# Maxwell-Zhao/RoboSimGS

Measured on AMD Instinct MI355X. Metric: frames/sec + ms/frame (fwd, fwd+bwd) at 1M Gaussians 1920x1080, higher is better.
Workload: dtype f32

## Files before the change

robosimgs_amd/csrc/binning.hip:

```cpp
#include "mgs_common.h"
#include "tile_rect.h"
#include "tile_order.h"

namespace mgs {
namespace {

constexpr int kBlock = 128;

__device__ __forceinline__ uint32_t wave_sum(uint32_t v) {
#pragma unroll
  for (int d = 32; d >= 1; d >>= 1) v += __shfl_xor(v, d);
  return v;
}

constexpr int kSum = 64;
__global__ __launch_bounds__(kBlock) void tile_count_kernel(
    int n, const float* __restrict__ means2d, const int32_t* __restrict__ radii,
    const int32_t* __restrict__ radii_y, const float* __restrict__ conics, const float* __restrict__ opacities,
    float tile_size, int tile_w, int tile_h, uint2* __restrict__ ginfo, uint32_t* __restrict__ sums) {
  int g = blockIdx.x * kBlock + threadIdx.x;
  int radius = g < n ? radii[g] : 0;
  uint2 info = make_uint2(kEmptyTileRect, 0u);
  if (radius > 0) {
    float2 m = reinterpret_cast<const float2*>(means2d)[g];
// ... 319 lines not shown
  uint32_t kept[kColKeep];
  uint32_t sum = 0;
  if (kCanKeep && keep) {
#pragma unroll
    for (int j = 0; j < kColKeep; ++j) {
      if (j >= rpg) { kept[j] = 0u; continue; }
      kept[j] = (ok && r0 + j < r1) ? table[(size_t)(r0 + j) * n_tiles + t] : 0u;
    }
#pragma unroll
    for (int j = 0; j < kColKeep; ++j) sum += kept[j];
  } else {
    for (int r = r0; r < r1; r += 16) {
      uint32_t v[16];
#pragma unroll
      for (int j = 0; j < 16; ++j) v[j] = (ok && r + j < r1) ? table[(size_t)(r + j) * n_tiles + t] : 0u;
#pragma unroll
      for (int j = 0; j < 16; ++j) sum += v[j];
    }
  }
  part[rg][bl] = sum;
  __syncthreads();
  uint32_t off = 0, tot = 0;
#pragma unroll 16
  for (int g = 0; g < kColGroups; ++g) {
    const uint32_t s = part[g][bl];
    if (g < rg) off += s;
    tot += s;
  }
  if (kCanKeep && keep) {
#pragma unroll
    for (int j = 0; j < kColKeep; ++j) {
      if (j >= rpg) continue;
      if (ok && r0 + j < r1) {
        table[(size_t)(r0 + j) * n_tiles + t] = off;
        off += kept[j];
      }
    }
  } else {
    for (int r = r0; r < r1; r += 16) {
      uint32_t v[16];
#pragma unroll
      for (int j = 0; j < 16; ++j) v[j] = (ok && r + j < r1) ? table[(size_t)(r + j) * n_tiles + t] : 0u;
#pragma unroll
      for (int j = 0; j < 16; ++j)
        if (ok && r + j < r1) {
          table[(size_t)(r + j) * n_tiles + t] = off;
          off += v[j];
        }
    }
  }
  if (rg == 0 && ok) tile_count[t] = tot;
}

template <bool PAIRS>
__global__ __launch_bounds__(kDirectThreads) void direct_scatter_kernel(
    int n, int chunk, const uint2* __restrict__ ginfo, int tile_w, int n_tiles, int shift,
    const uint32_t* __restrict__ table, const uint32_t* __restrict__ tile_count, uint32_t capacity,
    uint32_t* __restrict__ flatten_ids, int32_t* __restrict__ tile_offsets,
    uint32_t* __restrict__ n_isect, uint32_t* __restrict__ status, int32_t* __restrict__ group_order,
    const uint32_t* __restrict__ scanned_sums, int4* __restrict__ pair_info, uint32_t* __restrict__ zero_word,
    float* __restrict__ splat_slots, int deal_nb) {
  extern __shared__ uint32_t cursor[];
  n_tiles = (n_tiles + (1 << shift) - 1) >> shift;
  if (group_order && blockIdx.x == gridDim.x - 1) {
    order_groups_by_total<kDirectThreads>(n_tiles, [&](int g) { return tile_count[g]; }, group_order);
    return;
  }
  const uint32_t local_mask = (1u << shift) - 1u;
  __shared__ unsigned long long wsum[kDirectThreads / 64];
  const unsigned lane = threadIdx.x & 63, wave = threadIdx.x >> 6;
  const int per = (n_tiles + kDirectThreads - 1) / kDirectThreads;
  const int t0 = (int)threadIdx.x * per;
  unsigned long long sum = 0;
  for (int k = 0; k < per; ++k)
    if (t0 + k < n_tiles) sum += tile_count[t0 + k];
  unsigned long long incl = sum;
#pragma unroll
  for (int d = 1; d < 64; d <<= 1) {
    const uint32_t lo = __shfl_up((uint32_t)incl, d), hi = __shfl_up((uint32_t)(incl >> 32), d);
    if (lane >= (unsigned)d) incl += ((unsigned long long)hi << 32) | lo;
  }
  if (lane == 63) wsum[wave] = incl;
  __syncthreads();
  unsigned long long off = 0, total = 0;
#pragma unroll
  for (int w = 0; w < kDirectThreads / 64; ++w) {
    if ((unsigned)w < wave) off += wsum[w];
    total += wsum[w];
  }
  unsigned long long ex = off + incl - sum;
  const uint32_t* row = table + (size_t)blockIdx.x * n_tiles;
  for (int k = 0; k < per; ++k) {
    const int t = t0 + k;
    if (t < n_tiles) {
      const uint32_t at = ex < capacity ? (uint32_t)ex : capacity;
      cursor[t] = ex < capacity ? at + row[t] : capacity;
      if (blockIdx.x == 0) tile_offsets[t] = (int32_t)at;
      ex += tile_count[t];
    }
  }
  if (blockIdx.x == 0 && threadIdx.x == 0) {
    tile_offsets[n_tiles] = (int32_t)(total < capacity ? (uint32_t)total : capacity);
    *n_isect = total > 0xffffffffull ? 0xffffffffu : (uint32_t)total;
    *status = total > capacity ? MGS_STATUS_ISECT_OVERFLOW : 0u;
    if (zero_word) reinterpret_cast<uint4*>(zero_word)[0] = reinterpret_cast<uint4*>(zero_word)[1] = make_uint4(0u, 0u, 0u, 0u);
  }
  __syncthreads();
  const int g0 = blockIdx.x * chunk, g1 = min(n, g0 + chunk);
  const DealtIndex gi{g0, g1, n, deal_nb};
  const int g_end = deal_nb > 0 ? g0 + chunk : g1;
  for (int base = g0; base < g_end; base += kDirectThreads * kDirectPerThread) {
    uint2 info[kDirectPerThread];
#pragma unroll
    for (int i = 0; i < kDirectPerThread; ++i) {
      const int g = gi(base, i);
      info[i] = g >= 0 ? ginfo[g] : make_uint2(kEmptyTileRect, 0u);
    }
    if (PAIRS) {
// ... 56 lines not shown
  if (i0 + kOffsetsPerThread <= n) {
    const uint4 a = *reinterpret_cast<const uint4*>(tiles + i0), b = *reinterpret_cast<const uint4*>(tiles + i0 + 4);
    v[0] = a.x; v[1] = a.y; v[2] = a.z; v[3] = a.w; v[4] = b.x; v[5] = b.y; v[6] = b.z; v[7] = b.w;
  } else {
#pragma unroll
    for (int j = 0; j < kOffsetsPerThread; ++j) v[j] = i0 + j < n ? tiles[i0 + j] : 0u;
  }
  int prev = i0 ? (int)tiles[i0 - 1] : -1;
#pragma unroll
  for (int j = 0; j < kOffsetsPerThread; ++j) {
    const uint32_t i = i0 + j;
    if (i < n) {
      const int cur = (int)v[j];
      for (int k = prev + 1; k <= cur; ++k) offsets[k] = (int32_t)i;
      prev = cur;
      if (i == n - 1)
        for (int k = cur + 1; k <= n_tiles; ++k) offsets[k] = (int32_t)n;
    }
  }
}

__global__ __launch_bounds__(kBlock) void isect_ids_kernel(
    const uint32_t* __restrict__ n_ptr, uint32_t capacity, const uint32_t* __restrict__ tiles,
    const int32_t* __restrict__ ids, const float* __restrict__ depths, int64_t cam_shifted,
    int64_t* __restrict__ isect_ids) {
  uint32_t n = min(*n_ptr, capacity);
  uint32_t i = blockIdx.x * kBlock + threadIdx.x;
  if (i >= n) return;
  int64_t hi = cam_shifted | (int64_t)tiles[i];
  isect_ids[i] = (hi << 32) | (int64_t)__float_as_uint(depths[ids[i]]);
}

__global__ __launch_bounds__(kBlock) void offset_encode_kernel(
    uint32_t n, const int64_t* __restrict__ isect_ids, int n_cams, int n_tiles, int tile_bits,
    int32_t* __restrict__ offsets) {
  uint32_t i = blockIdx.x * kBlock + threadIdx.x;
  int total = n_cams * n_tiles;
  if (n == 0) {
    for (uint32_t k = i; k < (uint32_t)total; k += gridDim.x * kBlock) offsets[k] = 0;
    return;
  }
  if (i >= n) return;
  auto flat = [&](int64_t key) {
    int64_t t = key >> 32;
    return (int)((t >> tile_bits) * n_tiles + (t & ((1ll << tile_bits) - 1)));
  };
  int cur = flat(isect_ids[i]);
  int prev = i ? flat(isect_ids[i - 1]) : -1;
  for (int k = prev + 1; k <= cur && k < total; ++k) offsets[k] = (int32_t)i;
  if (i == n - 1)
    for (int k = cur + 1; k < total; ++k) offsets[k] = (int32_t)n;
}

__global__ __launch_bounds__(1024) void tile_group_order_kernel(int n_tiles, const int32_t* __restrict__ tile_offsets,
                                                                int32_t* __restrict__ order) {
  order_groups_by_total<1024>((n_tiles + 3) / 4, [&](int g) {
    return (uint32_t)(tile_offsets[min(4 * g + 4, n_tiles)] - tile_offsets[4 * g]);
  }, order);
}

int bits_for(uint32_t count) {
  int b = 0;
  while (count > 1 && (1ull << b) < count) ++b;
  return b;
}

unsigned direct_chunk(unsigned n) {
  const unsigned per_block = max(div_up(n, kDirectMaxBlocks), (unsigned)(kDirectThreads * kDirectPerThread));
  return div_up(per_block, kDirectThreads) * kDirectThreads;
}
unsigned direct_blocks(unsigned n) { return div_up(n, direct_chunk(n)); }

struct Workspace {
  size_t total;
  size_t ginfo, blocksums, tile_alt, tile_priv, id_alt, radix, tsort, table, tile_count, group_offsets;
  Workspace(int n, uint32_t cap, int n_tiles) {
    Bump b(0);
    size_t nn = (size_t)(n > 0 ? n : 1), cc = cap ? cap : 1;
    ginfo = b.take(nn * 8);
    blocksums = b.take((size_t)div_up((unsigned)nn, kSum) * 4);
    tile_alt = b.take(cc * 4); id_alt = b.take(cc * 4);
    tile_priv = b.take(cc * 4);
    radix = b.take(radix_sort_temp_bytes((uint32_t)cc));
    tsort = b.take(tile_depth_sort_temp_bytes((uint32_t)cc, n_tiles));
    const size_t nt = (size_t)(n_tiles < kDirectMaxTiles ? n_tiles : kDirectMaxTiles);
    table = b.take((size_t)direct_blocks((unsigned)nn) * nt * 4);
    tile_count = b.take(nt * 4);
    group_offsets = b.take((nt + 1) * 4);
    total = b.total;
  }
};

}
}

namespace mgs {
size_t isect_tiles_workspace_bytes(int n, uint32_t capacity, int n_tiles) { return Workspace(n, capacity, n_tiles).total; }

int launch_tile_group_order(int n_tiles, const int32_t* tile_offsets, int32_t* order, hipStream_t stream) {
  hipLaunchKernelGGL(tile_group_order_kernel, dim3(1), dim3(1024), 0, stream, n_tiles, tile_offsets, order);
  return check_launch("tile_group_order");
}
}

using namespace mgs;

extern "C" int mgs_isect_tiles(int n, const float* means2d, const int32_t* radii, const int32_t* radii_y,
                               const float* depths, const float* conics, const float* opacities,
                               int tile_size, int tile_w, int tile_h,
                               int cam_id, int n_cams, uint32_t isect_capacity,
                               int32_t* tiles_per_gauss, uint32_t* n_isect, uint32_t* tile_ids,
                               int32_t* flatten_ids, int64_t* isect_ids, int32_t* tile_offsets,
                               int32_t* pair_info, int32_t* tile_group_order, uint32_t* status,
                               const uint32_t* seed_info,
                               uint32_t* seed_sums, float* splat_slots, void* workspace,
                               size_t* workspace_bytes, mgs_stream_t stream) {
  MGS_REQUIRE(n >= 0 && tile_size > 0 && tile_w > 0 && tile_h > 0, "isect_tiles: bad sizes");
  MGS_REQUIRE(tile_w <= 1023 && tile_h <= 1023, "isect_tiles: tile grid %dx%d exceeds 1023x1023", tile_w, tile_h);
  MGS_REQUIRE(workspace_bytes, "isect_tiles: workspace_bytes is null");
  MGS_REQUIRE(cam_id >= 0 && n_cams > cam_id, "isect_tiles: cam_id %d outside 0..%d", cam_id, n_cams);
  const Workspace ws(n, isect_capacity, tile_w * tile_h);
  if (!workspace) {
    *workspace_bytes = ws.total;
    return MGS_OK;
  }
  if (*workspace_bytes < ws.total)
    return set_error(MGS_ERR_WORKSPACE_TOO_SMALL, "isect_tiles: workspace %zu < %zu bytes",
                     *workspace_bytes, ws.total);
  MGS_REQUIRE(isect_capacity > 0, "isect_tiles: zero capacity");
  MGS_REQUIRE(seed_info || (conics == nullptr) == (opacities == nullptr),
              "isect_tiles: tight tile bounds need both conics and opacities");
  MGS_REQUIRE(n == 0 || (seed_info == nullptr) == (seed_sums == nullptr),
              "isect_tiles: seed_info and seed_sums come together (mgs_project_color_fwd writes both)");
  MGS_REQUIRE((n == 0 || ((seed_info || (means2d && radii)) && depths)) && n_isect && flatten_ids &&
                  tile_offsets && status, "isect_tiles: null pointer");
  MGS_REQUIRE(!seed_info || tile_size == MGS_TILE_SIZE, "isect_tiles: a seed is for tile_size %d, got %d", MGS_TILE_SIZE, tile_size);
  MGS_REQUIRE(!seed_sums || (reinterpret_cast<uintptr_t>(seed_sums) & 15u) == 0, "isect_tiles: seed_sums must be 16-byte aligned");
  MGS_REQUIRE(!splat_slots || pair_info, "isect_tiles: splat_slots are written with pair_info");
  MGS_REQUIRE(!splat_slots || (reinterpret_cast<uintptr_t>(splat_slots) & 15u) == 0, "isect_tiles: splat_slots must be 16-byte aligned");
  hipStream_t s = (hipStream_t)stream;
  char* w = static_cast<char*>(workspace);
  auto u32 = [&](size_t off) { return reinterpret_cast<uint32_t*>(w + off); };
  const bool want_tile_ids = tile_ids != nullptr;
  if (!tile_ids) tile_ids = u32(ws.tile_priv);
  const int n_tiles = tile_w * tile_h;
  const uint32_t cap = isect_capacity;
  const int gshift = (sort_opts() & 8) ? (sort_opts() >> 4) & 7 : kGroupShift;
  const bool direct = ((n_tiles + (1 << gshift) - 1) >> gshift) <= kDirectMaxTiles && !(sort_opts() & 4) &&
                      (gshift == 0 || (unsigned)n <= (1u << (32 - gshift)));
  int rc;
  bool order_done = false;

  if (n == 0) {
    (void)hipMemsetAsync(n_isect, 0, 4, s);
    (void)hipMemsetAsync(status, 0, 4, s);
  } else {
    const unsigned nblk = div_up(n, kBlock), nsum = div_up(n, kSum);
    const uint2* ginfo = reinterpret_cast<const uint2*>(seed_info);
    uint32_t* sums = seed_sums;
    if (!seed_info) {
      uint2* gi = reinterpret_cast<uint2*>(w + ws.ginfo);
      sums = u32(ws.blocksums);
      hipLaunchKernelGGL(tile_count_kernel, dim3(nblk), dim3(kBlock), 0, s, n, means2d, radii, radii_y, conics,
                         opacities, (float)tile_size, tile_w, tile_h, gi, sums);
      ginfo = gi;
    }
    if (direct) {
      const int chunk = (int)direct_chunk((unsigned)n);
      const unsigned nb = direct_blocks((unsigned)n);
      const int bins = (n_tiles + (1 << gshift) - 1) >> gshift;
      const size_t lds = (size_t)bins * sizeof(uint32_t);
      const int deal_nb = (int)nb;
      hipLaunchKernelGGL(direct_hist_kernel, dim3(nb + (pair_info ? 1 : 0)), dim3(kDirectThreads), lds, s, n, chunk, ginfo, tile_w,
                         n_tiles, gshift, u32(ws.table), tiles_per_gauss, pair_info ? sums : nullptr, nsum, deal_nb);
      if (pair_info)
        hipLaunchKernelGGL(direct_colscan_kernel<kColKeepTraining>, dim3(div_up((unsigned)bins, (unsigned)kColBins)), dim3(kColThreads), 0, s,
                           (int)nb, bins, u32(ws.table), u32(ws.tile_count));
      else
        hipLaunchKernelGGL(direct_colscan_kernel<1>, dim3(div_up((unsigned)bins, (unsigned)kColBins)), dim3(kColThreads), 0, s,
                           (int)nb, bins, u32(ws.table), u32(ws.tile_count));
      const bool order_in_scatter = tile_group_order && gshift == 2;
      order_done = order_in_scatter;
      with_bool(pair_info != nullptr, [&](auto training) {
        hipLaunchKernelGGL(direct_scatter_kernel<decltype(training)::value>, dim3(nb + (order_in_scatter ? 1 : 0)),
                           dim3(kDirectThreads), lds, s, n, chunk, ginfo, tile_w, n_tiles, gshift, u32(ws.table),
                           u32(ws.tile_count), cap, gshift ? u32(ws.id_alt) : reinterpret_cast<uint32_t*>(flatten_ids),
                           gshift ? reinterpret_cast<int32_t*>(w + ws.group_offsets) : tile_offsets, n_isect, status,
                           order_in_scatter ? tile_group_order : nullptr, sums, reinterpret_cast<int4*>(pair_info),
                           tile_depth_sort_long_list(w + ws.tsort, cap), pair_info ? splat_slots : nullptr, deal_nb);
      });
    } else {
      hipLaunchKernelGGL(scan_blocksums_kernel, dim3(1), dim3(kScanThreads), 0, s, nsum, sums, cap,
                         n_isect, status);
      const int tile_bits = bits_for((uint32_t)n_tiles);
      const int passes = (tile_bits + 7) / 8;
      uint32_t* user_t = tile_ids;
      uint32_t* user_i = reinterpret_cast<uint32_t*>(flatten_ids);
      uint32_t *a_t = user_t, *a_i = user_i, *b_t = u32(ws.tile_alt), *b_i = u32(ws.id_alt);
      if (passes & 1) { a_t = u32(ws.tile_alt); a_i = u32(ws.id_alt); b_t = user_t; b_i = user_i; }
      hipLaunchKernelGGL(emit_kernel, dim3(nblk), dim3(kBlock), 0, s, n, ginfo, tile_w, sums, cap, a_t,
                         a_i, tiles_per_gauss);
      if (pair_info)
        hipLaunchKernelGGL(pair_info_kernel, dim3(nblk), dim3(kBlock), 0, s, n, ginfo, tile_h, sums,
                           reinterpret_cast<int4*>(pair_info), splat_slots);
      rc = radix_sort_pairs(n_isect, cap, tile_bits, a_t, a_i, b_t, b_i, w + ws.radix, s);
      if (rc) return rc;
    }
  }
  if (!direct || n == 0)
    hipLaunchKernelGGL(tile_offsets_kernel, dim3(div_up(cap, kBlock * kOffsetsPerThread)), dim3(kBlock), 0,
                       s, n_isect, cap, tile_ids, n_tiles, tile_offsets);
  if (n > 0) {
    const bool grouped = direct && gshift > 0;
    rc = tile_depth_sort(n_tiles, tile_offsets, depths, cap, reinterpret_cast<uint32_t*>(flatten_ids),
                         direct && (want_tile_ids || isect_ids) ? tile_ids : nullptr, w + ws.tsort, s,
                          u32(ws.tile_alt), u32(ws.id_alt),
                         grouped ? u32(ws.id_alt) : nullptr,
                         grouped ? reinterpret_cast<const int32_t*>(w + ws.group_offsets) : nullptr, gshift, direct);
    if (rc) return rc;
  }
  if (tile_group_order && !order_done) {
    rc = launch_tile_group_order(n_tiles, tile_offsets, tile_group_order, s);
    if (rc) return rc;
  }
  const unsigned gblk = div_up(cap, kBlock);
  if (isect_ids) {
    const int tile_bits_key = bits_for((uint32_t)n_tiles + 1);
    hipLaunchKernelGGL(isect_ids_kernel, dim3(gblk), dim3(kBlock), 0, s, n_isect, cap, tile_ids,
                       flatten_ids, depths, (int64_t)cam_id << tile_bits_key, isect_ids);
  }
  return check_launch("isect_tiles");
}

extern "C" int mgs_isect_offset_encode(uint32_t n_isect, const int64_t* isect_ids, int n_cams,
                                       int tile_w, int tile_h, int32_t* offsets,
                                       mgs_stream_t stream) {
  MGS_REQUIRE(n_cams > 0 && tile_w > 0 && tile_h > 0, "isect_offset_encode: bad sizes");
  MGS_REQUIRE(offsets && (isect_ids || n_isect == 0), "isect_offset_encode: null pointer");
  const int n_tiles = tile_w * tile_h;
  const int tile_bits = bits_for((uint32_t)n_tiles + 1);
  unsigned gblk = n_isect ? div_up(n_isect, kBlock) : div_up((unsigned)(n_cams * n_tiles), kBlock);
  hipLaunchKernelGGL(offset_encode_kernel, dim3(gblk), dim3(kBlock), 0, (hipStream_t)stream,
                     n_isect, isect_ids, n_cams, n_tiles, tile_bits, offsets);
// ... 3 lines not shown
```

robosimgs_amd/csrc/labels.hip:

```cpp
#include "weight_walk.h"
#include "tile_order.h"
#include "../../include/mgs_labels.h"

namespace mgs {
namespace {

__global__ __launch_bounds__(64) void raster_labels_kernel(
    const float* __restrict__ means2d, const float* __restrict__ conics, const float* __restrict__ opacities,
    const float4* __restrict__ splats, const int32_t* __restrict__ class_ids, int n_classes, int width, int height,
    int tile_w, int n_tiles, const int32_t* __restrict__ tile_offsets, const int32_t* __restrict__ flatten_ids,
    const int32_t* __restrict__ group_order, uint8_t* __restrict__ labels, float* __restrict__ label_weights) {
  __shared__ WeightEntry queue[kQueue + 1];
  extern __shared__ __attribute__((aligned(16))) float class_w[];
  const int tile = tile_of_unit((int)blockIdx.x, n_tiles, group_order);
  if (tile < 0) return;
  const unsigned lane = threadIdx.x & 63u;
  const TileFrame fr = tile_frame(tile, tile_w, lane);
  const int start = tile_offsets[tile], end = tile_offsets[tile + 1];
  const int ix = fr.ix, iy = fr.iy;
  if (start >= end) {
#pragma unroll
    for (int k = 0; k < 4; ++k) {
      const int x = ix + 8 * (k & 1), y = iy + 8 * (k >> 1);
      if (x < width && y < height) {
        const size_t p = (size_t)y * width + x;
        labels[p] = MGS_LABEL_NONE;
        if (label_weights) label_weights[p] = 0.f;
      }
    }
    return;
  }

  for (int i = 0; i < n_classes; ++i)
    reinterpret_cast<float4*>(class_w)[i * 64 + lane] = make_float4(0.f, 0.f, 0.f, 0.f);

  unsigned long long alive[4];
#pragma unroll
  for (int k = 0; k < 4; ++k)
    alive[k] = ballot(ix + 8 * (k & 1) < width && iy + 8 * (k >> 1) < height);
  __builtin_amdgcn_fence(__ATOMIC_RELEASE, "wavefront");
  __builtin_amdgcn_wave_barrier();
  __builtin_amdgcn_fence(__ATOMIC_ACQUIRE, "wavefront");

  weight_walk(queue, fr, lane, start, end, splats, means2d, conics, opacities, flatten_ids, alive,
              [&](int g) { return class_ids[g]; },
              [&](int cls, auto quad) {
                const bool counted = (unsigned)cls < (unsigned)n_classes;
                float* slot = class_w + (counted ? cls : 0) * 256 + lane;
#pragma unroll
                for (int k = 0; k < 4; ++k) {
                  float w;
                  if (quad(k, w) && counted) atomicAdd(slot + 64 * k, w);
                }
              });

  __builtin_amdgcn_fence(__ATOMIC_RELEASE, "wavefront");
  __builtin_amdgcn_wave_barrier();
  __builtin_amdgcn_fence(__ATOMIC_ACQUIRE, "wavefront");
  float best[4] = {0.f, 0.f, 0.f, 0.f};
  int label[4] = {MGS_LABEL_NONE, MGS_LABEL_NONE, MGS_LABEL_NONE, MGS_LABEL_NONE};
  for (int c = 0; c < n_classes; ++c) {
#pragma unroll
    for (int k = 0; k < 4; ++k) {
      const float v = class_w[c * 256 + 64 * k + lane];
      if (v > best[k]) { best[k] = v; label[k] = c; }
    }
  }
#pragma unroll
  for (int k = 0; k < 4; ++k) {
    const int x = ix + 8 * (k & 1), y = iy + 8 * (k >> 1);
    if (x < width && y < height) {
      const size_t p = (size_t)y * width + x;
      labels[p] = (uint8_t)label[k];
      if (label_weights) label_weights[p] = best[k];
    }
  }
}

}

int check_label_args(const char* fn, const int32_t* class_ids, int n_classes, const uint8_t* labels) {
  MGS_REQUIRE(n_classes >= 1 && n_classes <= MGS_LABELS_MAX_CLASSES, "%s: n_classes %d outside 1..%d", fn, n_classes,
              MGS_LABELS_MAX_CLASSES);
  MGS_REQUIRE(class_ids, "%s: class_ids is null", fn);
  MGS_REQUIRE(labels, "%s: labels is null", fn);
  return MGS_OK;
}

}

using namespace mgs;

extern "C" int mgs_raster_labels(int n, const float* means2d, const float* conics, const float* opacities,
                                 const float* splats, const int32_t* class_ids, int n_classes, int width, int height,
                                 int tile_w, int tile_h, const int32_t* tile_offsets, const int32_t* flatten_ids,
                                 const int32_t* tile_group_order, uint8_t* labels, float* label_weights,
                                 mgs_stream_t stream) {
  const int rc = check_label_args("raster_labels", class_ids, n_classes, labels);
  if (rc) return rc;
  MGS_REQUIRE(splats || (means2d && conics && opacities),
              "raster_labels: neither packed records (splats) nor means2d, conics and opacities given");
  MGS_REQUIRE(n >= 0 && width > 0 && height > 0, "raster_labels: bad sizes");
  MGS_REQUIRE(tile_w == (width + 15) / 16 && tile_h == (height + 15) / 16,
              "raster_labels: tile grid %dx%d does not match %dx%d at tile size 16", tile_w, tile_h, width, height);
  MGS_REQUIRE(tile_offsets && flatten_ids, "raster_labels: null tile lists");
  const int n_tiles = tile_w * tile_h, n_units = tile_launch_units(n_tiles, tile_group_order);
  hipLaunchKernelGGL(raster_labels_kernel, dim3(n_units), dim3(64), (size_t)n_classes * 1024, (hipStream_t)stream, means2d,
                     conics, opacities, reinterpret_cast<const float4*>(splats), class_ids, n_classes, width, height, tile_w,
                     n_tiles, tile_offsets, flatten_ids, tile_group_order, labels, label_weights);
  return check_launch("raster_labels");
}
```

robosimgs_amd/csrc/lift.hip:

```cpp
#include "weight_walk.h"
#include "tile_order.h"
#include "../../include/mgs_lift.h"

#include <math.h>

namespace mgs {
namespace {

constexpr float kVoteOne = 4294967296.f;

__global__ __launch_bounds__(64) void raster_votes_kernel(
    const float* __restrict__ means2d, const float* __restrict__ conics, const float* __restrict__ opacities,
    const float4* __restrict__ splats, const uint8_t* __restrict__ mask, int n_classes, int width, int height, int tile_w,
    int n_tiles, const int32_t* __restrict__ tile_offsets, const int32_t* __restrict__ flatten_ids,
    const int32_t* __restrict__ group_order, int row_offset, int n_rows, unsigned long long* __restrict__ votes) {
  __shared__ WeightEntry queue[kQueue + 1];
  const int tile = tile_of_unit((int)blockIdx.x, n_tiles, group_order);
  if (tile < 0) return;
  const unsigned lane = threadIdx.x & 63u;
  const int start = tile_offsets[tile], end = tile_offsets[tile + 1];
  if (start >= end) return;
  const TileFrame fr = tile_frame(tile, tile_w, lane);

  unsigned cls_of[4];
  unsigned have = 0u;
#pragma unroll
  for (int k = 0; k < 4; ++k) {
    const int x = fr.ix + 8 * (k & 1), y = fr.iy + 8 * (k >> 1);
    unsigned m = 255u;
    if (x < width && y < height) m = mask[(size_t)y * width + x];
    if (m >= (unsigned)n_classes) m = 255u;
    else have |= 1u << m;
    cls_of[k] = m;
  }
  const unsigned mask4 = cls_of[0] | cls_of[1] << 8 | cls_of[2] << 16 | cls_of[3] << 24;
  const unsigned present = wave_or(have);
  if (present == 0u) return;

  unsigned long long alive[4];
#pragma unroll
  for (int k = 0; k < 4; ++k) alive[k] = ballot(((mask4 >> (8 * k)) & 255u) != 255u);

  weight_walk(queue, fr, lane, start, end, splats, means2d, conics, opacities, flatten_ids, alive,
              [&](int g) { return g - row_offset; },
              [&](int row, auto quad) {
                float w[4] = {0.f, 0.f, 0.f, 0.f};
#pragma unroll
                for (int k = 0; k < 4; ++k) quad(k, w[k]);
                if ((unsigned)row >= (unsigned)n_rows) return;
                if (ballot((w[0] + w[1]) + (w[2] + w[3]) > 0.f) == 0ull) return;
                unsigned long long* dst = votes + (size_t)row * (size_t)n_classes;
                unsigned todo = present;
                while (todo != 0u) {
                  const unsigned c = (unsigned)__builtin_ctz(todo);
                  todo &= todo - 1u;
                  float s[4];
#pragma unroll
                  for (int k = 0; k < 4; ++k) s[k] = ((mask4 >> (8 * k)) & 255u) == c ? w[k] : 0.f;
                  const float sum = wave_reduce_to_lane63((s[0] + s[1]) + (s[2] + s[3]));
                  if (lane == 63u && sum > 0.f)
                    atomicAdd(dst + c, (unsigned long long)rintf(sum * kVoteOne));
                }
              });
}

__global__ __launch_bounds__(256) void lift_assign_kernel(int n_rows, int n_classes,
                                                          const unsigned long long* __restrict__ votes,
                                                          unsigned long long min_vote, int32_t* __restrict__ class_ids,
                                                          float* __restrict__ confidence) {
  const int g = (int)(blockIdx.x * 256u + threadIdx.x);
  if (g >= n_rows) return;
  const unsigned long long* v = votes + (size_t)g * (size_t)n_classes;
  unsigned long long best = 0ull, total = 0ull;
  int cls = 0;
  for (int c = 0; c < n_classes; ++c) {
    const unsigned long long x = v[c];
    total += x;
    if (x > best) { best = x; cls = c; }
  }
  const bool assigned = best > min_vote;
  class_ids[g] = assigned ? cls : -1;
  if (confidence) confidence[g] = assigned ? (float)((double)best / (double)total) : 0.f;
}

}
}

using namespace mgs;

extern "C" int mgs_raster_votes(int n, const float* means2d, const float* conics, const float* opacities,
                                const float* splats, const uint8_t* mask, int n_classes, int width, int height, int tile_w,
                                int tile_h, const int32_t* tile_offsets, const int32_t* flatten_ids,
                                const int32_t* tile_group_order, int row_offset, int n_rows, uint64_t* votes,
                                mgs_stream_t stream) {
  MGS_REQUIRE(n_classes >= 1 && n_classes <= MGS_LABELS_MAX_CLASSES, "raster_votes: n_classes %d outside 1..%d", n_classes,
              MGS_LABELS_MAX_CLASSES);
  MGS_REQUIRE(mask, "raster_votes: mask is null");
  MGS_REQUIRE(votes, "raster_votes: votes is null");
  MGS_REQUIRE(n_rows >= 0, "raster_votes: n_rows %d is negative", n_rows);
  MGS_REQUIRE(splats || (means2d && conics && opacities),
              "raster_votes: neither packed records (splats) nor means2d, conics and opacities given");
  MGS_REQUIRE(n >= 0 && width > 0 && height > 0, "raster_votes: bad sizes");
  MGS_REQUIRE(tile_w == (width + 15) / 16 && tile_h == (height + 15) / 16,
              "raster_votes: tile grid %dx%d does not match %dx%d at tile size 16", tile_w, tile_h, width, height);
  MGS_REQUIRE(tile_offsets && flatten_ids, "raster_votes: null tile lists");
  const int n_tiles = tile_w * tile_h, n_units = tile_launch_units(n_tiles, tile_group_order);
  hipLaunchKernelGGL(raster_votes_kernel, dim3(n_units), dim3(64), 0, (hipStream_t)stream, means2d, conics, opacities,
                     reinterpret_cast<const float4*>(splats), mask, n_classes, width, height, tile_w, n_tiles, tile_offsets,
                     flatten_ids, tile_group_order, row_offset, n_rows, reinterpret_cast<unsigned long long*>(votes));
  return check_launch("raster_votes");
}

extern "C" int mgs_lift_assign(int n_rows, int n_classes, const uint64_t* votes, float min_vote, int32_t* class_ids,
                               float* confidence, mgs_stream_t stream) {
  MGS_REQUIRE(n_rows >= 0, "lift_assign: n_rows %d is negative", n_rows);
  MGS_REQUIRE(n_classes >= 1 && n_classes <= MGS_LABELS_MAX_CLASSES, "lift_assign: n_classes %d outside 1..%d", n_classes,
              MGS_LABELS_MAX_CLASSES);
  MGS_REQUIRE(votes, "lift_assign: votes is null");
  MGS_REQUIRE(class_ids, "lift_assign: class_ids is null");
  MGS_REQUIRE(min_vote >= 0.f && min_vote < 2147483648.f, "lift_assign: min_vote %g outside 0 <= min_vote < 2^31",
              (double)min_vote);
  if (n_rows == 0) return MGS_OK;
  const unsigned long long min_q = (unsigned long long)rint((double)min_vote * 4294967296.0);
  hipLaunchKernelGGL(lift_assign_kernel, dim3(div_up((unsigned)n_rows, 256u)), dim3(256), 0, (hipStream_t)stream, n_rows,
                     n_classes, reinterpret_cast<const unsigned long long*>(votes), min_q, class_ids, confidence);
  return check_launch("lift_assign");
}
```

robosimgs_amd/csrc/raster_fwd.hip:

```cpp
#include <type_traits>

#include "raster_common.h"
#include "tile_order.h"
#include "dataset_pixel.h"

namespace mgs {
namespace {

constexpr int kFwdMinWaves = 5;
constexpr int kFwdWgWaves = 4;

template <int CHT>
struct QueueEntry {
  float4 geo0;
  float4 geo1;
  float4 feat[(CHT + 3) / 4];
  float4 geo3;
};

template <int CHT>
struct PixelState {
  float T;
  float C[CHT];
  int last;
// ... 305 lines not shown
          entry(e[2]);
          if (rest == 0ull) break;
          entry(e[3]);
          if (rest == 0ull) break;
        }
      } else {
        do entry(*e++); while (rest != 0ull);
      }
    };
    if (all_safe) walk(std::true_type{}); else walk(std::false_type{});
    __builtin_amdgcn_wave_barrier();
  }

#ifdef MGS_RASTER_STATS
  {
    unsigned nv = 0, na = 0;
    for (int k = 0; k < 4; ++k) { nv += st[k].n_valid; na += st[k].n_acc; }
    for (int d = 32; d >= 1; d >>= 1) { nv += __shfl_xor(nv, d); na += __shfl_xor(na, d); }
    stat[3] = nv; stat[4] = na;
    if (lane == 0)
      for (int i = 0; i < 7; ++i) atomicAdd(&g_raster_stats[i], stat[i]);
  }
#endif
  if constexpr (TRACK_LAST) {
    if (ckpt) {
      int h = max(max(st[0].last, st[1].last), max(st[2].last, st[3].last));
#pragma unroll
      for (int d = 32; d >= 1; d >>= 1) h = max(h, __shfl_xor(h, d));
      if (lane < 4) reinterpret_cast<int32_t*>(ckpt)[4 * tile + lane] = lane == 0 ? h : -1;
    }
  }
#pragma unroll
  for (int k = 0; k < 4; ++k) {
    const int x = ix + 8 * (k & 1), y = iy + 8 * (k >> 1);
    if (x < width && y < height)
      store_pixel<CHT, TRACK_LAST, DATASET>(st[k], x, y, width, channels, background, expected_last, render, alphas, last_ids, ds);
  }
}


template <int CHT, bool TRACK_LAST, bool DATASET = false>
__global__ __launch_bounds__(256) void raster_fwd_q_kernel(
    const float* __restrict__ means2d, const float* __restrict__ conics,
    const float* __restrict__ feats, const float* __restrict__ opacities,
    const float4* __restrict__ splats, const float* __restrict__ background, int channels,
    int width, int height, int tile_w, int n_tiles, const int32_t* __restrict__ tile_offsets,
    const int32_t* __restrict__ flatten_ids, float* __restrict__ render,
    float* __restrict__ alphas, int32_t* __restrict__ last_ids, int cull, int expected_last,
    const int32_t* __restrict__ group_order, float* __restrict__ ckpt, int ckpt_shift,
    std::conditional_t<DATASET, DatasetOut, NoDataset> ds) {
  __shared__ QueueEntry<CHT> queues[4][kQueue];
  const int k = (int)(threadIdx.x >> 6);
  QueueEntry<CHT>* queue = queues[k];
  const int tile = tile_of_unit(blockIdx.x, n_tiles, group_order);
  if (tile < 0) return;
  const unsigned lane = threadIdx.x & 63u;
  const int tx = tile % tile_w, ty = tile / tile_w;
  const int start = tile_offsets[tile], end = tile_offsets[tile + 1];
  const int ix = tx * 16 + 8 * (k & 1) + (int)(lane & 7), iy = ty * 16 + 8 * (k >> 1) + (int)(lane >> 3);
  const PixelPoly pp = pixel_poly((float)(8 * (k & 1) + (int)(lane & 7)) - 7.5f, (float)(8 * (k >> 1) + (int)(lane >> 3)) - 7.5f);
  const bool inside = ix < width && iy < height;
  QuadRect rect;
  rect.x0 = (float)(tx * 16 + 8 * (k & 1)) + 0.5f; rect.x1 = rect.x0 + 7.f;
  rect.y0 = (float)(ty * 16 + 8 * (k >> 1)) + 0.5f; rect.y1 = rect.y0 + 7.f;
  const float tile_x = (float)(tx * 16), tile_y = (float)(ty * 16);

  PixelState<CHT> st;
  st.T = (inside || kMasks<CHT>) ? 1.f : -1.f;
  unsigned long long alive = ballot(inside);
  st.last = 0;
#pragma unroll
  for (int c = 0; c < CHT; ++c) st.C[c] = 0.f;

  int r_idx = start + (int)lane;
  bool r_ok = r_idx < end;
  float2 r_xy = make_float2(0.f, 0.f);
  float r_ca = 1.f, r_cb = 0.f, r_cc = 1.f, r_op = 0.f;
  float r_feat[CHT];
#pragma unroll
  for (int c = 0; c < CHT; ++c) r_feat[c] = 0.f;
  auto fetch = [&](int idx, bool ok) {
    if (ok && CHT <= 4 && splats) {
      int g = flatten_ids[idx];
      const float4 p0 = splats[3 * (size_t)g], p1 = splats[3 * (size_t)g + 1], p2 = splats[3 * (size_t)g + 2];
      r_xy = make_float2(p0.x, p0.y);
      r_ca = p0.z; r_cb = p0.w; r_cc = p1.x; r_op = p1.y;
      const float ff[4] = {p1.z, p1.w, p2.x, p2.y};
#pragma unroll
      for (int c = 0; c < CHT; ++c) r_feat[c] = ff[c & 3];
    } else if (ok) {
      int g = flatten_ids[idx];
      r_xy = reinterpret_cast<const float2*>(means2d)[g];
      r_ca = conics[3 * (size_t)g + 0];
      r_cb = conics[3 * (size_t)g + 1];
      r_cc = conics[3 * (size_t)g + 2];
      r_op = opacities[g];
#pragma unroll
      for (int c = 0; c < CHT; ++c) r_feat[c] = c < channels ? feats[(size_t)g * channels + c] : 0.f;
    }
  };
  fetch(r_idx, r_ok);

  for (int b = start; b < end; b += kQueue) {
    if ((kMasks<CHT> ? alive : ballot(st.T > 0.f)) == 0ull) break;
    if constexpr (TRACK_LAST) {
      if (ckpt && b != start && ((b - start) & ((1 << ckpt_shift) - 1)) == 0) {
        float* cp = ckpt + ckpt_header_floats(n_tiles) + ckpt_unit(start, tile, (b - start) >> ckpt_shift, ckpt_shift) * (size_t)(1 + channels) * 256 + 64 * k + lane;
// ... 116 lines not shown
}
#endif

extern "C" size_t mgs_raster_checkpoint_floats(uint32_t isect_capacity, int tile_w, int tile_h, int channels,
                                               int checkpoint_interval) {
  if (checkpoint_interval < 64 || (checkpoint_interval & (checkpoint_interval - 1)) || tile_w <= 0 || tile_h <= 0 || channels < 1)
    return 0;
  int shift = 0;
  while ((1 << shift) < checkpoint_interval) ++shift;
  return ckpt_header_floats(tile_w * tile_h) + ckpt_units(isect_capacity, tile_w * tile_h, shift) * (size_t)(1 + channels) * 256;
}

extern "C" int mgs_rasterize_fwd(int n, const float* means2d, const float* conics,
                                 const float* feats, const float* opacities, const float* splats,
                                 const float* background, int channels, int width, int height,
                                 int tile_w, int tile_h, const int32_t* tile_offsets,
                                 const int32_t* flatten_ids, const int32_t* tile_group_order, int flags,
                                 float* render, float* alphas, int32_t* last_ids, float* checkpoints,
                                 int checkpoint_interval, uint8_t* ds_rgba, void* ds_distance, int ds_distance_type,
                                 const double* ds_Kinv_host, mgs_stream_t stream) {
  MGS_REQUIRE(n >= 0 && width > 0 && height > 0, "rasterize_fwd: bad sizes");
  MGS_REQUIRE(channels >= 1 && channels <= MGS_MAX_CHANNELS, "rasterize_fwd: channels %d outside 1..%d", channels, MGS_MAX_CHANNELS);
  MGS_REQUIRE(tile_w == (width + 15) / 16 && tile_h == (height + 15) / 16,
              "rasterize_fwd: tile grid %dx%d does not match %dx%d at tile size 16", tile_w, tile_h, width, height);
  MGS_REQUIRE(!splats || channels <= 4, "rasterize_fwd: packed splats carry at most 4 channels");
  MGS_REQUIRE((n == 0 || splats || (means2d && conics && feats && opacities)) && tile_offsets &&
                  flatten_ids && ((render && alphas) || (ds_rgba && !render && !alphas)), "rasterize_fwd: null pointer");
  DatasetOut ds{};
  if (ds_rgba || ds_distance) {
    MGS_REQUIRE(ds_rgba && channels == 4 && (flags & MGS_RASTER_EXPECTED_LAST) && !last_ids,
                "rasterize_fwd: the dataset output needs ds_rgba, 4 channels, MGS_RASTER_EXPECTED_LAST and no last_ids");
    MGS_REQUIRE(((uintptr_t)ds_rgba & 3) == 0, "rasterize_fwd: ds_rgba must be 4-byte aligned");
    MGS_REQUIRE(!ds_distance || ds_Kinv_host, "rasterize_fwd: the distance map needs K^-1 (host pointer, 9 doubles)");
    MGS_REQUIRE(ds_distance_type >= 0 && ds_distance_type <= 2, "rasterize_fwd: distance type %d not in {0: f32, 1: f64, 2: f16}",
                ds_distance_type);
    ds.rgba = reinterpret_cast<uint32_t*>(ds_rgba);
    ds.dist = ds_distance;
    ds.type = ds_distance_type;
    for (int i = 0; i < 9; ++i) ds.ki.m[i] = ds_Kinv_host ? ds_Kinv_host[i] : 0.0;
  }
  int ckpt_shift = 0;
  if (checkpoints) {
    MGS_REQUIRE(last_ids, "rasterize_fwd: checkpoints are written by the training variant (last_ids given)");
    MGS_REQUIRE(checkpoint_interval >= 64 && (checkpoint_interval & (checkpoint_interval - 1)) == 0,
                "rasterize_fwd: checkpoint_interval %d is not a power of two >= 64", checkpoint_interval);
    while ((1 << ckpt_shift) < checkpoint_interval) ++ckpt_shift;
  }
  const int n_tiles = tile_w * tile_h;
  hipStream_t s = (hipStream_t)stream;
  const bool per_block = (g_raster_opts & 4) || ((g_raster_opts & 2) && (flags & MGS_RASTER_LATENCY));
  if (g_raster_opts & 8) tile_group_order = nullptr;
  if ((g_raster_opts & 16) && !per_block && !last_ids) tile_group_order = nullptr;
  const int n_units = tile_launch_units(n_tiles, tile_group_order);
  const int expected_last = (flags & MGS_RASTER_EXPECTED_LAST) ? 1 : 0;
  const size_t opts_lds = (size_t)(g_raster_opts >> 8) * 1024;
  auto launch = [&](auto cht, auto track_last, auto ds_arg) {
    constexpr int C = decltype(cht)::value;
    constexpr bool T = decltype(track_last)::value, DS = std::is_same<decltype(ds_arg), DatasetOut>::value;
    if (per_block && C <= 4) {
      hipLaunchKernelGGL((raster_fwd_q_kernel<C, T, DS>), dim3(n_units), dim3(256), opts_lds, s, means2d, conics, feats,
                         opacities, reinterpret_cast<const float4*>(splats), background, channels, width, height, tile_w,
                         n_tiles, tile_offsets, flatten_ids, render, alphas, last_ids, g_raster_cull, expected_last,
                         tile_group_order, checkpoints, ckpt_shift, ds_arg);
      return;
    }
    hipLaunchKernelGGL((raster_fwd_kernel<C, T, DS>), dim3(div_up(n_units, T ? 1 : kFwdWgWaves)),
                       dim3(64 * (T ? 1 : kFwdWgWaves)), T ? 0 : opts_lds, s, means2d, conics, feats, opacities,
                       reinterpret_cast<const float4*>(splats), background, channels, width, height, tile_w, n_tiles,
                       tile_offsets, flatten_ids, render, alphas, last_ids, g_raster_cull, expected_last, g_raster_opts,
                       tile_group_order, checkpoints, ckpt_shift, ds_arg);
  };
  if (ds.rgba) launch(int_c<4>{}, bool_c<false>{}, ds);
  else
    with_channels(channels, [&](auto cht) { with_bool(last_ids != nullptr, [&](auto t) { launch(cht, t, NoDataset{}); }); });
  return check_launch("rasterize_fwd");
}
```

robosimgs_amd/csrc/tile_order.h:

```cpp
#ifndef MGS_TILE_ORDER_H_
#define MGS_TILE_ORDER_H_

#include "mgs_common.h"

namespace mgs {

constexpr int kOrderClasses = 1024;

template <int T, class Total>
__device__ __forceinline__ void order_groups_by_total(int n_groups, Total total, int32_t* __restrict__ order) {
  __shared__ uint32_t hist[kOrderClasses];
  __shared__ uint32_t wave_tot[T / 64];
  __shared__ uint32_t longest;
  constexpr int kPer = kOrderClasses / T;
  constexpr int kBatch = 8;
  const int t = threadIdx.x;
#pragma unroll
  for (int k = 0; k < kPer; ++k) hist[t * kPer + k] = 0u;
  if (t == 0) longest = 1u;
  __syncthreads();
  uint32_t m = 1u;
  for (int g0 = 0; g0 < n_groups; g0 += T * kBatch) {
    uint32_t v[kBatch];
#pragma unroll
    for (int j = 0; j < kBatch; ++j) v[j] = g0 + j * T + t < n_groups ? total(g0 + j * T + t) : 0u;
#pragma unroll
    for (int j = 0; j < kBatch; ++j) m = max(m, v[j]);
  }
#pragma unroll
  for (int d = 32; d >= 1; d >>= 1) m = max(m, (uint32_t)__shfl_xor((int)m, d));
  if ((t & 63) == 0) atomicMax(&longest, m);
  __syncthreads();
  const float scale = (float)(kOrderClasses - 1) / (float)longest;
  auto cls = [&](uint32_t len) {
    return kOrderClasses - 1 - min(kOrderClasses - 1, (int)((float)len * scale));
  };
  for (int g0 = 0; g0 < n_groups; g0 += T * kBatch) {
    uint32_t v[kBatch];
#pragma unroll
    for (int j = 0; j < kBatch; ++j) v[j] = g0 + j * T + t < n_groups ? total(g0 + j * T + t) : 0u;
#pragma unroll
    for (int j = 0; j < kBatch; ++j)
      if (g0 + j * T + t < n_groups) atomicAdd(&hist[cls(v[j])], 1u);
  }
  __syncthreads();
  uint32_t c[kPer], sum = 0;
#pragma unroll
  for (int k = 0; k < kPer; ++k) { c[k] = hist[t * kPer + k]; sum += c[k]; }
  uint32_t incl = sum;
#pragma unroll
  for (int d = 1; d < 64; d <<= 1) {
    const uint32_t up = __shfl_up(incl, d);
    if ((t & 63) >= d) incl += up;
  }
  if ((t & 63) == 63) wave_tot[t >> 6] = incl;
  __syncthreads();
  uint32_t ex = incl - sum;
  for (int w = 0; w < (t >> 6); ++w) ex += wave_tot[w];
#pragma unroll
  for (int k = 0; k < kPer; ++k) { hist[t * kPer + k] = ex; ex += c[k]; }
  __syncthreads();
  for (int g0 = 0; g0 < n_groups; g0 += T * kBatch) {
    uint32_t v[kBatch];
#pragma unroll
    for (int j = 0; j < kBatch; ++j) v[j] = g0 + j * T + t < n_groups ? total(g0 + j * T + t) : 0u;
#pragma unroll
    for (int j = 0; j < kBatch; ++j)
      if (g0 + j * T + t < n_groups) order[atomicAdd(&hist[cls(v[j])], 1u)] = g0 + j * T + t;
  }
}

__device__ __forceinline__ int tile_of_unit(int unit, int n_tiles, const int32_t* __restrict__ group_order) {
  if (!group_order) return unit < n_tiles ? unit : -1;
  if (unit >= ((n_tiles + 3) & ~3)) return -1;
  const int tile = group_order[unit >> 2] * 4 + (unit & 3);
  return tile < n_tiles ? tile : -1;
}

inline int tile_launch_units(int n_tiles, const int32_t* group_order) { return group_order ? (n_tiles + 3) / 4 * 4 : n_tiles; }

int launch_tile_group_order(int n_tiles, const int32_t* tile_offsets, int32_t* order, hipStream_t stream);

}
#endif
```

Before: 4601.

## Deal tile groups across XCD regions and interleave raster block-to-tile mapping

```diff
diff --git a/robosimgs_amd/csrc/binning.hip b/robosimgs_amd/csrc/binning.hip
--- a/robosimgs_amd/csrc/binning.hip
+++ b/robosimgs_amd/csrc/binning.hip
@@ -395,7 +395,7 @@
   if (rg == 0 && ok) tile_count[t] = tot;
 }
 
-template <bool PAIRS>
+template <bool PAIRS, bool REGIONS>
 __global__ __launch_bounds__(kDirectThreads) void direct_scatter_kernel(
     int n, int chunk, const uint2* __restrict__ ginfo, int tile_w, int n_tiles, int shift,
     const uint32_t* __restrict__ table, const uint32_t* __restrict__ tile_count, uint32_t capacity,
@@ -406,7 +406,12 @@
   extern __shared__ uint32_t cursor[];
   n_tiles = (n_tiles + (1 << shift) - 1) >> shift;
   if (group_order && blockIdx.x == gridDim.x - 1) {
-    order_groups_by_total<kDirectThreads>(n_tiles, [&](int g) { return tile_count[g]; }, group_order);
+    static_assert(kDirectMaxTiles <= kOrderMaxStaged, "the order's stage is the scatter's cursor array");
+    if constexpr (REGIONS)
+      order_groups_by_total<kDirectThreads>(n_tiles, [&](int g) { return tile_count[g]; }, group_order,
+                                            reinterpret_cast<int32_t*>(cursor));
+    else
+      order_groups_plain<kDirectThreads>(n_tiles, [&](int g) { return tile_count[g]; }, group_order);
     return;
   }
   const uint32_t local_mask = (1u << shift) - 1u;
@@ -569,11 +574,13 @@
     for (int k = cur + 1; k < total; ++k) offsets[k] = (int32_t)n;
 }
 
+template <bool REGIONS>
 __global__ __launch_bounds__(1024) void tile_group_order_kernel(int n_tiles, const int32_t* __restrict__ tile_offsets,
                                                                 int32_t* __restrict__ order) {
-  order_groups_by_total<1024>((n_tiles + 3) / 4, [&](int g) {
-    return (uint32_t)(tile_offsets[min(4 * g + 4, n_tiles)] - tile_offsets[4 * g]);
-  }, order);
+  extern __shared__ int32_t order_stage[];
+  auto total = [&](int g) { return (uint32_t)(tile_offsets[min(4 * g + 4, n_tiles)] - tile_offsets[4 * g]); };
+  if constexpr (REGIONS) order_groups_by_total<1024>((n_tiles + 3) / 4, total, order, order_stage);
+  else order_groups_plain<1024>((n_tiles + 3) / 4, total, order);
 }
 
 int bits_for(uint32_t count) {
@@ -615,7 +622,12 @@
 size_t isect_tiles_workspace_bytes(int n, uint32_t capacity, int n_tiles) { return Workspace(n, capacity, n_tiles).total; }
 
 int launch_tile_group_order(int n_tiles, const int32_t* tile_offsets, int32_t* order, hipStream_t stream) {
-  hipLaunchKernelGGL(tile_group_order_kernel, dim3(1), dim3(1024), 0, stream, n_tiles, tile_offsets, order);
+  const int n_groups = (n_tiles + 3) / 4, staged = order_regions() && n_groups <= kOrderMaxStaged;
+  if (staged)
+    hipLaunchKernelGGL(tile_group_order_kernel<true>, dim3(1), dim3(1024), (size_t)n_groups * sizeof(int32_t), stream,
+                       n_tiles, tile_offsets, order);
+  else
+    hipLaunchKernelGGL(tile_group_order_kernel<false>, dim3(1), dim3(1024), 0, stream, n_tiles, tile_offsets, order);
   return check_launch("tile_group_order");
 }
 }
@@ -698,14 +710,14 @@
                            (int)nb, bins, u32(ws.table), u32(ws.tile_count));
       const bool order_in_scatter = tile_group_order && gshift == 2;
       order_done = order_in_scatter;
-      with_bool(pair_info != nullptr, [&](auto training) {
-        hipLaunchKernelGGL(direct_scatter_kernel<decltype(training)::value>, dim3(nb + (order_in_scatter ? 1 : 0)),
+      with_bool(pair_info != nullptr, [&](auto training) { with_bool(order_regions(), [&](auto regions) {
+        hipLaunchKernelGGL((direct_scatter_kernel<decltype(training)::value, decltype(regions)::value>), dim3(nb + (order_in_scatter ? 1 : 0)),
                            dim3(kDirectThreads), lds, s, n, chunk, ginfo, tile_w, n_tiles, gshift, u32(ws.table),
                            u32(ws.tile_count), cap, gshift ? u32(ws.id_alt) : reinterpret_cast<uint32_t*>(flatten_ids),
                            gshift ? reinterpret_cast<int32_t*>(w + ws.group_offsets) : tile_offsets, n_isect, status,
                            order_in_scatter ? tile_group_order : nullptr, sums, reinterpret_cast<int4*>(pair_info),
                            tile_depth_sort_long_list(w + ws.tsort, cap), pair_info ? splat_slots : nullptr, deal_nb);
-      });
+      }); });
     } else {
       hipLaunchKernelGGL(scan_blocksums_kernel, dim3(1), dim3(kScanThreads), 0, s, nsum, sums, cap,
                          n_isect, status);
diff --git a/robosimgs_amd/csrc/labels.hip b/robosimgs_amd/csrc/labels.hip
--- a/robosimgs_amd/csrc/labels.hip
+++ b/robosimgs_amd/csrc/labels.hip
@@ -12,7 +12,7 @@
     const int32_t* __restrict__ group_order, uint8_t* __restrict__ labels, float* __restrict__ label_weights) {
   __shared__ WeightEntry queue[kQueue + 1];
   extern __shared__ __attribute__((aligned(16))) float class_w[];
-  const int tile = tile_of_unit((int)blockIdx.x, n_tiles, group_order);
+  const int tile = tile_of_unit_xcd((int)blockIdx.x, n_tiles, group_order);
   if (tile < 0) return;
   const unsigned lane = threadIdx.x & 63u;
   const TileFrame fr = tile_frame(tile, tile_w, lane);
@@ -104,7 +104,7 @@
   MGS_REQUIRE(tile_w == (width + 15) / 16 && tile_h == (height + 15) / 16,
               "raster_labels: tile grid %dx%d does not match %dx%d at tile size 16", tile_w, tile_h, width, height);
   MGS_REQUIRE(tile_offsets && flatten_ids, "raster_labels: null tile lists");
-  const int n_tiles = tile_w * tile_h, n_units = tile_launch_units(n_tiles, tile_group_order);
+  const int n_tiles = tile_w * tile_h, n_units = tile_launch_units_xcd(n_tiles, tile_group_order);
   hipLaunchKernelGGL(raster_labels_kernel, dim3(n_units), dim3(64), (size_t)n_classes * 1024, (hipStream_t)stream, means2d,
                      conics, opacities, reinterpret_cast<const float4*>(splats), class_ids, n_classes, width, height, tile_w,
                      n_tiles, tile_offsets, flatten_ids, tile_group_order, labels, label_weights);
diff --git a/robosimgs_amd/csrc/lift.hip b/robosimgs_amd/csrc/lift.hip
--- a/robosimgs_amd/csrc/lift.hip
+++ b/robosimgs_amd/csrc/lift.hip
@@ -15,7 +15,7 @@
     int n_tiles, const int32_t* __restrict__ tile_offsets, const int32_t* __restrict__ flatten_ids,
     const int32_t* __restrict__ group_order, int row_offset, int n_rows, unsigned long long* __restrict__ votes) {
   __shared__ WeightEntry queue[kQueue + 1];
-  const int tile = tile_of_unit((int)blockIdx.x, n_tiles, group_order);
+  const int tile = tile_of_unit_xcd((int)blockIdx.x, n_tiles, group_order);
   if (tile < 0) return;
   const unsigned lane = threadIdx.x & 63u;
   const int start = tile_offsets[tile], end = tile_offsets[tile + 1];
@@ -104,7 +104,7 @@
   MGS_REQUIRE(tile_w == (width + 15) / 16 && tile_h == (height + 15) / 16,
               "raster_votes: tile grid %dx%d does not match %dx%d at tile size 16", tile_w, tile_h, width, height);
   MGS_REQUIRE(tile_offsets && flatten_ids, "raster_votes: null tile lists");
-  const int n_tiles = tile_w * tile_h, n_units = tile_launch_units(n_tiles, tile_group_order);
+  const int n_tiles = tile_w * tile_h, n_units = tile_launch_units_xcd(n_tiles, tile_group_order);
   hipLaunchKernelGGL(raster_votes_kernel, dim3(n_units), dim3(64), 0, (hipStream_t)stream, means2d, conics, opacities,
                      reinterpret_cast<const float4*>(splats), mask, n_classes, width, height, tile_w, n_tiles, tile_offsets,
                      flatten_ids, tile_group_order, row_offset, n_rows, reinterpret_cast<unsigned long long*>(votes));
diff --git a/robosimgs_amd/csrc/raster_fwd.hip b/robosimgs_amd/csrc/raster_fwd.hip
--- a/robosimgs_amd/csrc/raster_fwd.hip
+++ b/robosimgs_amd/csrc/raster_fwd.hip
@@ -381,7 +381,7 @@
   __shared__ QueueEntry<CHT> queues[4][kQueue];
   const int k = (int)(threadIdx.x >> 6);
   QueueEntry<CHT>* queue = queues[k];
-  const int tile = tile_of_unit(blockIdx.x, n_tiles, group_order);
+  const int tile = tile_of_unit_xcd(blockIdx.x, n_tiles, group_order);
   if (tile < 0) return;
   const unsigned lane = threadIdx.x & 63u;
   const int tx = tile % tile_w, ty = tile / tile_w;
@@ -604,13 +604,14 @@
   if (g_raster_opts & 8) tile_group_order = nullptr;
   if ((g_raster_opts & 16) && !per_block && !last_ids) tile_group_order = nullptr;
   const int n_units = tile_launch_units(n_tiles, tile_group_order);
+  const int n_units_q = tile_launch_units_xcd(n_tiles, tile_group_order);
   const int expected_last = (flags & MGS_RASTER_EXPECTED_LAST) ? 1 : 0;
   const size_t opts_lds = (size_t)(g_raster_opts >> 8) * 1024;
   auto launch = [&](auto cht, auto track_last, auto ds_arg) {
     constexpr int C = decltype(cht)::value;
     constexpr bool T = decltype(track_last)::value, DS = std::is_same<decltype(ds_arg), DatasetOut>::value;
     if (per_block && C <= 4) {
-      hipLaunchKernelGGL((raster_fwd_q_kernel<C, T, DS>), dim3(n_units), dim3(256), opts_lds, s, means2d, conics, feats,
+      hipLaunchKernelGGL((raster_fwd_q_kernel<C, T, DS>), dim3(n_units_q), dim3(256), opts_lds, s, means2d, conics, feats,
                          opacities, reinterpret_cast<const float4*>(splats), background, channels, width, height, tile_w,
                          n_tiles, tile_offsets, flatten_ids, render, alphas, last_ids, g_raster_cull, expected_last,
                          tile_group_order, checkpoints, ckpt_shift, ds_arg);
diff --git a/robosimgs_amd/csrc/tile_order.h b/robosimgs_amd/csrc/tile_order.h
--- a/robosimgs_amd/csrc/tile_order.h
+++ b/robosimgs_amd/csrc/tile_order.h
@@ -3,12 +3,106 @@
 
 #include "mgs_common.h"
 
+#ifndef MGS_TO_HD
+#define MGS_TO_HD __host__ __device__ __forceinline__
+#endif
+
 namespace mgs {
 
 constexpr int kOrderClasses = 1024;
-
+constexpr int kOrderRegions = 8;
+constexpr int kRegionClasses = kOrderClasses / kOrderRegions;
+constexpr uint32_t kOrderMaxTotal = 1u << 29;
+constexpr int kOrderMaxStaged = 15000;
+
+struct DealPlan {
+  int n[kOrderRegions];
+  int sur[kOrderRegions];
+  int lvl[kOrderRegions + 1];
+  int above[kOrderRegions + 1];
+};
+
+MGS_TO_HD DealPlan deal_plan(int n_groups, const int* cut) {
+  DealPlan d;
+#pragma unroll
+  for (int r = 0; r < kOrderRegions; ++r) {
+    d.n[r] = cut[r + 1] - cut[r];
+    const int slots = (n_groups - r + 7) >> 3;
+    d.sur[r] = d.n[r] > slots ? d.n[r] - slots : 0;
+  }
+#pragma unroll
+  for (int m = 0; m <= kOrderRegions; ++m) d.lvl[m] = 0;
+#pragma unroll
+  for (int r = 0; r < kOrderRegions; ++r) {
+    int rank = 0;
+#pragma unroll
+    for (int q = 0; q < kOrderRegions; ++q) rank += (d.sur[q] > d.sur[r] || (d.sur[q] == d.sur[r] && q < r)) ? 1 : 0;
+#pragma unroll
+    for (int m = 0; m < kOrderRegions; ++m) d.lvl[m] += rank == m ? d.sur[r] : 0;
+  }
+  d.above[0] = 0;
+#pragma unroll
+  for (int m = 1; m <= kOrderRegions; ++m) d.above[m] = d.above[m - 1] + m * (d.lvl[m - 1] - d.lvl[m]);
+  return d;
+}
+
+MGS_TO_HD void deal_source(const DealPlan& d, int p, int& region, int& k) {
+  const int round = p >> 3, slot = p & 7;
+  int f = 0;
+#pragma unroll
+  for (int s = 0; s < kOrderRegions; ++s) {
+    const int c = ((p + 7 - s) >> 3) - d.n[s];
+    f += c > 0 ? c : 0;
+  }
+  int v = 0, w = 0;
+#pragma unroll
+  for (int m = kOrderRegions; m >= 1; --m)
+    if (f < d.above[m] && f >= d.above[m - 1]) {
+      const int in = f - d.above[m - 1];
+      v = d.lvl[m - 1] - in / m;
+      w = in % m;
+    }
+  int n_own = 0, own_handed = 0, giver = 0, giver_handed = 0, idx = 0;
+#pragma unroll
+  for (int r = 0; r < kOrderRegions; ++r) {
+    const bool at_level = v > 0 && d.sur[r] >= v;
+    const int handed = (d.sur[r] > v ? d.sur[r] - v : 0) + (at_level && idx < w ? 1 : 0);
+    if (at_level && idx == w) { giver = r; giver_handed = handed; }
+    if (r == slot) { n_own = d.n[r]; own_handed = handed; }
+    idx += at_level ? 1 : 0;
+  }
+  if (round < n_own) {
+    region = slot;
+    k = round + own_handed;
+  } else {
+    region = giver;
+    k = ((p + 7 - giver) >> 3) + giver_handed;
+  }
+}
+
+MGS_TO_HD int tile_of_unit(int unit, int n_tiles, const int32_t* __restrict__ group_order) {
+  if (!group_order) return unit < n_tiles ? unit : -1;
+  if (unit >= ((n_tiles + 3) & ~3)) return -1;
+  const int tile = group_order[unit >> 2] * 4 + (unit & 3);
+  return tile < n_tiles ? tile : -1;
+}
+
+inline int tile_launch_units(int n_tiles, const int32_t* group_order) { return group_order ? (n_tiles + 3) / 4 * 4 : n_tiles; }
+
+MGS_TO_HD int tile_of_unit_xcd(int unit, int n_tiles, const int32_t* __restrict__ group_order) {
+  if (!group_order) return unit < n_tiles ? unit : -1;
+  const int pos = (unit >> 5) * 8 + (unit & 7);
+  if (pos >= (n_tiles + 3) >> 2) return -1;
+  const int tile = group_order[pos] * 4 + ((unit >> 3) & 3);
+  return tile < n_tiles ? tile : -1;
+}
+inline int tile_launch_units_xcd(int n_tiles, const int32_t* group_order) {
+  return group_order ? ((n_tiles + 3) / 4 + 7) / 8 * 32 : n_tiles;
+}
+
+#if defined(__HIPCC__)
 template <int T, class Total>
-__device__ __forceinline__ void order_groups_by_total(int n_groups, Total total, int32_t* __restrict__ order) {
+__device__ __forceinline__ void order_groups_plain(int n_groups, Total total, int32_t* __restrict__ order) {
   __shared__ uint32_t hist[kOrderClasses];
   __shared__ uint32_t wave_tot[T / 64];
   __shared__ uint32_t longest;
@@ -70,16 +164,147 @@
   }
 }
 
-__device__ __forceinline__ int tile_of_unit(int unit, int n_tiles, const int32_t* __restrict__ group_order) {
-  if (!group_order) return unit < n_tiles ? unit : -1;
-  if (unit >= ((n_tiles + 3) & ~3)) return -1;
-  const int tile = group_order[unit >> 2] * 4 + (unit & 3);
-  return tile < n_tiles ? tile : -1;
-}
-
-inline int tile_launch_units(int n_tiles, const int32_t* group_order) { return group_order ? (n_tiles + 3) / 4 * 4 : n_tiles; }
+template <int T, class Total>
+__device__ __forceinline__ void order_groups_by_total(int n_groups, Total total, int32_t* __restrict__ order,
+                                                      int32_t* __restrict__ stage) {
+  __shared__ uint32_t hist[kOrderClasses];
+  __shared__ uint32_t wave_tot[T / 64];
+  __shared__ unsigned long long wave_sum[T / 64];
+  __shared__ uint32_t longest;
+  __shared__ int cut_s[kOrderRegions + 1];
+  constexpr int kPer = kOrderClasses / T;
+  constexpr int kBatch = 8;
+  const int t = threadIdx.x;
+#pragma unroll
+  for (int k = 0; k < kPer; ++k) hist[t * kPer + k] = 0u;
+  if (t == 0) longest = 1u;
+  if (t <= kOrderRegions) cut_s[t] = t ? n_groups : 0;
+  __syncthreads();
+  const int per = (n_groups + T - 1) / T;
+  const int g_lo = min(t * per, n_groups), g_hi = min(g_lo + per, n_groups);
+  const bool small = n_groups <= T * kBatch;
+  uint32_t run[kBatch], dealt[kBatch], left = 0u;
+#pragma unroll
+  for (int j = 0; j < kBatch; ++j) {
+    run[j] = small && g_lo + j < g_hi ? total(g_lo + j) : 0u;
+    dealt[j] = small && j * T + t < n_groups ? total(j * T + t) : 0u;
+  }
+  if (small && g_lo && g_lo < g_hi) left = total(g_lo - 1);
+  auto over_run = [&](auto f) {
+    if (small) {
+#pragma unroll
+      for (int j = 0; j < kBatch; ++j)
+        if (g_lo + j < g_hi) f(g_lo + j, run[j]);
+      return;
+    }
+    for (int g0 = g_lo; g0 < g_hi; g0 += kBatch) {
+      uint32_t v[kBatch];
+#pragma unroll
+      for (int j = 0; j < kBatch; ++j) v[j] = g0 + j < g_hi ? total(g0 + j) : 0u;
+#pragma unroll
+      for (int j = 0; j < kBatch; ++j)
+        if (g0 + j < g_hi) f(g0 + j, v[j]);
+    }
+  };
+  auto over_dealt = [&](auto f) {
+    if (small) {
+#pragma unroll
+      for (int j = 0; j < kBatch; ++j)
+        if (j * T + t < n_groups) f(j * T + t, dealt[j]);
+      return;
+    }
+    for (int g0 = 0; g0 < n_groups; g0 += T * kBatch) {
+      uint32_t v[kBatch];
+#pragma unroll
+      for (int j = 0; j < kBatch; ++j) v[j] = g0 + j * T + t < n_groups ? total(g0 + j * T + t) : 0u;
+#pragma unroll
+      for (int j = 0; j < kBatch; ++j)
+        if (g0 + j * T + t < n_groups) f(g0 + j * T + t, v[j]);
+    }
+  };
+  uint32_t m = 1u;
+  unsigned long long sum = 0;
+  over_run([&](int, uint32_t len) { m = max(m, len); sum += len; });
+#pragma unroll
+  for (int d = 32; d >= 1; d >>= 1) m = max(m, (uint32_t)__shfl_xor((int)m, d));
+  if ((t & 63) == 0) atomicMax(&longest, m);
+  unsigned long long incl64 = sum;
+#pragma unroll
+  for (int d = 1; d < 64; d <<= 1) {
+    const uint32_t lo = __shfl_up((uint32_t)incl64, d), hi = __shfl_up((uint32_t)(incl64 >> 32), d);
+    if ((t & 63) >= d) incl64 += ((unsigned long long)hi << 32) | lo;
+  }
+  if ((t & 63) == 63) wave_sum[t >> 6] = incl64;
+  __syncthreads();
+  unsigned long long before = incl64 - sum, all = 0;
+#pragma unroll 2
+  for (int w = 0; w < T / 64; ++w) {
+    if (w < (t >> 6)) before += wave_sum[w];
+    all += wave_sum[w];
+  }
+  const uint32_t all_hi = (uint32_t)__builtin_amdgcn_readfirstlane((int)(all >> 32));
+  const uint32_t s8 = (uint32_t)__builtin_amdgcn_readfirstlane((int)(uint32_t)all);
+  const bool regions = n_groups >= kOrderRegions && stage != nullptr && all_hi == 0u && s8 > 0u && s8 < kOrderMaxTotal;
+  if (regions && g_lo < g_hi) {
+    if (!small && g_lo) left = total(g_lo - 1);
+    uint32_t p8 = 8u * (uint32_t)before, last8 = p8 - 8u * left;
+    over_run([&](int g, uint32_t len) {
+#pragma unroll
+      for (uint32_t q = 1; q < (uint32_t)kOrderRegions; ++q)
+        if (p8 >= q * s8 && last8 < q * s8) cut_s[q] = g;
+      last8 = p8;
+      p8 += 8u * len;
+    });
+  }
+  __syncthreads();
+  int cut[kOrderRegions + 1];
+#pragma unroll
+  for (int r = 0; r <= kOrderRegions; ++r) cut[r] = __builtin_amdgcn_readfirstlane(cut_s[r]);
+  const int n_cls = regions ? kRegionClasses : kOrderClasses;
+  const float scale = (float)(n_cls - 1) / (float)(uint32_t)__builtin_amdgcn_readfirstlane((int)longest);
+  auto bin = [&](int g, uint32_t len) {
+    int r = 0;
+#pragma unroll
+    for (int q = 1; q < kOrderRegions; ++q) r += g >= cut[q] ? 1 : 0;
+    return r * kRegionClasses + n_cls - 1 - min(n_cls - 1, (int)((float)len * scale));
+  };
+  over_dealt([&](int g, uint32_t len) { atomicAdd(&hist[bin(g, len)], 1u); });
+  __syncthreads();
+  uint32_t c[kPer], csum = 0;
+#pragma unroll
+  for (int k = 0; k < kPer; ++k) { c[k] = hist[t * kPer + k]; csum += c[k]; }
+  uint32_t incl = csum;
+#pragma unroll
+  for (int d = 1; d < 64; d <<= 1) {
+    const uint32_t up = __shfl_up(incl, d);
+    if ((t & 63) >= d) incl += up;
+  }
+  if ((t & 63) == 63) wave_tot[t >> 6] = incl;
+  __syncthreads();
+  uint32_t ex = incl - csum;
+  for (int w = 0; w < (t >> 6); ++w) ex += wave_tot[w];
+#pragma unroll
+  for (int k = 0; k < kPer; ++k) { hist[t * kPer + k] = ex; ex += c[k]; }
+  __syncthreads();
+  int32_t* sorted = regions ? stage : order;
+  over_dealt([&](int g, uint32_t len) { sorted[atomicAdd(&hist[bin(g, len)], 1u)] = g; });
+  if (!regions) return;
+  __syncthreads();
+  const DealPlan plan = deal_plan(n_groups, cut);
+#pragma clang loop unroll(disable) vectorize(disable) interleave(disable)
+  for (int p = t; p < n_groups; p += T) {
+    int r, k;
+    deal_source(plan, p, r, k);
+#pragma unroll
+    for (int q = 0; q < kOrderRegions; ++q) k += q == r ? cut[q] : 0;
+    order[p] = stage[min(k, n_groups - 1)];
+  }
+}
+
+inline bool order_regions() { return (sort_opts() & 128) != 0; }
 
 int launch_tile_group_order(int n_tiles, const int32_t* tile_offsets, int32_t* order, hipStream_t stream);
-
-}
 #endif
+
+}
+#endif
```

Measured after the change: 4527. 1.6% lower.
